# Fytex/Shafa-CD

Hardware: AMD Instinct MI355X
Metric: GiB/s Shannon-Fano encode+decode, 64 MiB blocks, 1/2/4/8 GPUs; bit-exact (higher is better)
Workload: dtype u8

## Files before the change

shafa-cd_amd/csrc/sf_decode.hip:

```cpp
#include <type_traits>
#include "common.hpp"
#include "internal.hpp"

#include <atomic>
#include <mutex>
#include <thread>

#include <algorithm>

#include <stdlib.h>

#include "sfd_common.hpp"
#include "sfd_dp.hpp"
#include "sfd_generic.hpp"

namespace {

typedef __attribute__((address_space(3))) u32 lds_u32;
typedef __attribute__((address_space(3))) u16 lds_u16;
typedef __attribute__((address_space(3))) u8 lds_u8;
template <int LONG> constexpr u32 spec_emask() { return LONG == 2 ? 31u : 15u; }

constexpr int SC_PHW = 16;
constexpr int SC_M = 4;
// ... 725 lines not shown
    if (lds_addr(smem) != 0) __builtin_trap();
    const u32 units = (blk.n_tiles + SC_WTILES - 1) / SC_WTILES;
    u32 first_end = units - 1;
    if (units >= 2 && blk.in_n - (u64)(units - 2) * SC_WTILES * DTILE < (u64)64 * SC_SB + 4) first_end = units - 2;
    if (blockIdx.x > 0) {
        const u32 t_end = first_end * SC_WTILES, t_begin = 1u + (blockIdx.x - 1u) * SF_LINKS;
        if (t_begin < t_end)
            sf_links<LONG>(smem, blk, t_begin, t_end, chunk_entry, chunk_cnt, tile_cnt, tile_guess, tile_exit, tab_bytes, long_bytes);
        return;
    }
    fill_lds16((void *)(smem + SL_LDS_DATA), (const void *)blk.cnt3, 2u << blk.KW);
    if (LONG) {
        u16 *lt = (u16 *)(smem + SL_LDS_DATA + tab_bytes + SL_MISC);
        const u16 *src = LONG == 1 ? blk.longtab : blk.long32;
        if (src) fill_lds16((void *)lt, src, long_bytes);
        else if (threadIdx.x == 0) *lt = 0;
    }
    __syncthreads();
    u32 e0 = first_end ? (u32)tile_exit[(size_t)blk.tile_base + first_end * SC_WTILES - 1] : 0u;
    for (u32 u = first_end; u < units; ++u)
        e0 = sl_region<LONG>(smem, blk, u * SC_WTILES, e0, chunk_entry, chunk_cnt, tile_cnt, tile_guess, tile_exit, tab_bytes);
}

constexpr int ws_row(bool esc) { return CH_BYTES / 4 + (esc ? 3 : 2); }
constexpr int ws_rows_bytes(bool esc)
{
    return 16 + (DEC_THREADS * ws_row(esc) + (esc ? 0 : DEC_THREADS / 16)) * 4;
}
constexpr int WS_MISC = 32;
typedef unsigned int u32x3_t __attribute__((ext_vector_type(3)));
constexpr u32 WS_NST = 4, WS_DROP = 0x7FFFFFF0u;
constexpr int WS_RSRC_FLAGS = 0x00020000, WS_AUX_NT = 2;

template <int LONG, bool ESC>
__global__ __launch_bounds__(DEC_THREADS) void sfd_wstage(const DecBlk *__restrict__ blks, const u8 *__restrict__ chunk_entry,
                                                          const u16 *__restrict__ chunk_cnt, const u64 *__restrict__ tile_off,
                                                          u32 tpw, u32 tab_bytes, u32 cap, u32 long_bytes)
{
    extern __shared__ __attribute__((aligned(16))) u8 smem[];
    const DecBlk blk = blks[blockIdx.y];
    const u32 first_tile = blockIdx.x * tpw;
    if (first_tile >= blk.n_tiles) return;
    if (tile_off[(size_t)blk.tile_base + first_tile] >= blk.n_sym) return;
    const u32 LONGB = LONG ? long_bytes : 0u;
    u32 *rows = (u32 *)(smem + 16);
    constexpr u32 WS_ROW = (u32)ws_row(ESC), tab_off = (u32)ws_rows_bytes(ESC);
    const u16 *lt = (const u16 *)(smem + tab_off + tab_bytes);
    const u32 img_off = tab_off + tab_bytes + LONGB;
    u32 *wsum = (u32 *)(smem + img_off + cap);
    u32 *next = wsum + 4;
    const u32 tid = threadIdx.x, lane = tid & 63, wv = tid >> 6;
    const u32 K1 = blk.K1, K3 = sym3_window(K1);
    const u32 sh = 32 - K1;
    fill_lds16(smem + tab_off, (const void *)blk.sym3, 4u << K3);
    if (LONG) {
        const u16 *src = LONG == 1 ? blk.longtab : blk.long32;
        if (src) fill_lds16((void *)lt, src, LONGB);
        else if (tid == 0) *(u16 *)lt = 0;
    }
    for (u32 i = tid; i < cap / 16; i += DEC_THREADS) *(uint4 *)(smem + img_off + 16 * i) = make_uint4(0, 0, 0, 0);
    bool bad = false;
    if (lds_addr(smem) != 0) __builtin_trap();
    const u32 q2row = 8u * (16u + 4u * (WS_ROW * tid + (ESC ? 0u : tid >> 4))) - 2u;
    const u32 mask4 = ((1u << K3) - 1u) << 2;
    auto fetch16 = [&](const u64 off) -> uint4 {
        if (off + 16 <= blk.in_n) return gload_nt<uint4>(blk.in + off);
        u32 w[4] = {0, 0, 0, 0};
        if (off < blk.in_n) {
            const int nv = (int)(blk.in_n - off);
#pragma unroll
            for (int q = 0; q < 16; ++q)
                if (q < nv) w[q >> 2] |= (u32)gload<u8>(blk.in + off + q) << (8 * (q & 3));
        }
        return make_uint4(w[0], w[1], w[2], w[3]);
    };
    uint4 pf0, pf1;
    u32 pf2[ESC ? 3 : 2] = {};
    auto fetch_ahead = [&](const u64 off) {
        constexpr int NB = ESC ? 12 : 8;
        if (off + NB <= blk.in_n) {
            if constexpr (ESC) {
                const u32x3_t v = __builtin_nontemporal_load((const GLOBAL_AS u32x3_t *)(unsigned long long)(blk.in + off));
                pf2[0] = v.x; pf2[1] = v.y; pf2[2] = v.z;
            } else {
                const uint2 v = gload_nt<uint2>(blk.in + off);
                pf2[0] = v.x; pf2[1] = v.y;
            }
            return;
        }
        u32 w[3] = {0, 0, 0};
        if (off < blk.in_n) {
            const int nv = (int)(blk.in_n - off);
#pragma unroll
            for (int q = 0; q < NB; ++q)
                if (q < nv) w[q >> 2] |= (u32)gload<u8>(blk.in + off + q) << (8 * (q & 3));
        }
#pragma unroll
// ... 55 lines not shown
        u32 pre = incl - cnt, total = 0;
        for (u32 w = 0; w < 4; ++w) { if (w < wv) pre += wsum[w]; total += wsum[w]; }
        const u64 room = blk.n_sym - toff;
        const u32 tot_c = (u32)__builtin_amdgcn_readfirstlane((int)(room < (u64)total ? (u32)room : total));
        u32 want = pre >= tot_c ? 0u : (tot_c - pre < cnt ? tot_c - pre : cnt);
        u32 q2 = q2row + entry;
        const bool by_pos = want == cnt && tile + 1 < blk.n_tiles && nent != spec_emask<LONG>();
        const u32 q2end = q2row + 256u + nent;
        u32 done = 0;
        do {
            u8 *gout = blk.out + toff + done;
            const u32 mis = (u32)((uintptr_t)gout & 15u);
            if (carry_g && (carry_n != mis || carry_g != gout - mis)) {
                if (tid == 0) {
                    uint4 *ip = (uint4 *)(smem + img_off);
                    store_bytes(carry_g, *ip, carry_lo, carry_n);
                    ip[0] = make_uint4(0, 0, 0, 0);
                    ip[1] = make_uint4(0, 0, 0, 0);
                }
                carry_n = 0;
                carry_g = nullptr;
                lds_barrier();
            }
            const u32 capw = cap - 32;
            u32 nxt = tot_c;
            if (mis + (tot_c - done) > capw) {
                if (tid == 0) *next = tot_c;
                lds_barrier();
                if (want && pre >= done && mis + (pre - done) + want > capw) atomicMin(next, pre);
                lds_barrier();
                nxt = (u32)__builtin_amdgcn_readfirstlane((int)*next);
                lds_barrier();
            }
            if (want && pre >= done && pre + want <= nxt) {
                const u32 x = mis + (pre - done);
                u32 wp = img_off + (x & ~3u), nbx = x << 30, acc = 0;
                auto emit = [&](const u32 e) {
                    const u32 sh = nbx >> 27, syms = e & 0xFFFFFFu;
                    acc |= syms << sh;
                    if (__builtin_add_overflow(nbx, e & 0xC0000000u, &nbx)) {
                        __hip_atomic_fetch_or((lds_u32 *)(size_t)wp, acc, __ATOMIC_RELAXED, __HIP_MEMORY_SCOPE_WORKGROUP);
                        wp += 4u;
                        acc = syms >> (32u - sh);
                    }
                };
                auto window4 = [&]() -> u32 {
                    const lds_u32 *pa = (const lds_u32 *)(size_t)((q2 >> 3) & ~3u);
                    return __builtin_amdgcn_alignbit(pa[1], pa[0], q2);
                };
                auto step = [&](const bool tail) {
                    u32 e = *(const lds_u32 *)(size_t)(tab_off + (window4() & mask4));
                    if (ESC && __builtin_expect((e >> 30) == 0, 0)) {
                        const u32 q = q2 + 2u;
                        const lds_u32 *pb = (const lds_u32 *)(size_t)((q >> 3) & ~3u);
                        const u32 win = __builtin_bitreverse32(__builtin_amdgcn_alignbit(pb[1], pb[0], q));
                        u32 e1 = LONG == 1 ? long_code(lt, win) : LONG == 2 ? long_code32(lt, win)
                                           : (u32)gload<u16>(blk.lut13 + (win >> sh));
                        if (e1 == 0) { bad = true; e1 = 1u << 8; }
                        e = (e1 & 0xFFu) | ((e1 >> 8) << 24) | (1u << 30);
                    }
                    u32 n = e >> 30, syms = e & 0xFFFFFFu;
                    if (tail) {
                        n = n < want ? n : want;
                        syms &= (1u << (8 * n)) - 1u;
                    }
                    emit(syms | n << 30);
                    q2 += (e >> 24) & 63u;
// ... 176 lines not shown
    u64 rs = key | 1ull;
    int fails = 0;
    for (int trial = 0; trial < SPEC_TRIALS && fails <= SPEC_MAX_FAILS; ++trial) {
        u64 w[SPEC_WORDS];
        for (u64 &x : w) x = spec_rand(rs);
        if (!spec_trial(w, h.lenlut.data(), h.K1)) ++fails;
    }
    const bool yes = fails <= SPEC_MAX_FAILS;
    std::lock_guard<std::mutex> lk(cmu);
    ckey[slot] = key;
    cval[slot] = yes ? 2 : 1;
    return yes;
}

struct SfdArrays {
    u8 *cfn, *tfn;
    u8 *tent, *cent;
    u16 *ccnt;
    u32 *tcnt;
    u64 *toff;
    u8 *tguess, *texit;
};

enum SfdForm { SFD_MID32, SFD_LONG_ALL, SFD_PACKED12, SFD_PACKED13, SFD_PACKED };

static u32 sfd_tpw(u32 most, u32 max_tiles, int nblocks)
{
    u32 tpw = most;
    while (tpw > 1 && (u64)ceil_div_u64(max_tiles, tpw) * nblocks < 2048) tpw >>= 1;
    return tpw;
}

static void sfd_launch_packed(hipStream_t st, const DecBlk *dblk, int nblocks, u32 max_tiles, SfdForm form, bool esc, bool spec,
                              u32 tabb, u32 long_used, bool all_spec, u32 ws_tab, u32 ws_cap, const SfdArrays &a)
{
    static decltype(&sfd_scan<0>) const scans[3] = {sfd_scan<2>, sfd_scan<1>, sfd_scan<0>};
    static decltype(&sfd_ends<0>) const ends[3] = {sfd_ends<2>, sfd_ends<1>, sfd_ends<0>};
    static decltype(&sfd_sync16<true, false>) const syncs[4] = {sfd_sync16<false, true>, sfd_sync16<true, false, 12>,
                                                                sfd_sync16<true, false, 13>, sfd_sync16<true, false>};
    const int f = form < SFD_PACKED12 ? form : 2;
    const dim3 grid_b((u32)nblocks), wg(DEC_THREADS);
    hipLaunchKernelGGL(sfd_tables, dim3((u32)nblocks, 8), wg, 0, st, dblk);
    if (spec) {
        const size_t lds_scan = (size_t)SC_LDS_ROWS + tabb + SC_MISC + long_used;
        const size_t lds_ends = (size_t)SL_LDS_DATA + tabb + SL_MISC + long_used;
        hipLaunchKernelGGL(scans[f], dim3((u32)ceil_div_u64(max_tiles, SC_TILES), (u32)nblocks), wg, lds_scan, st, dblk, a.cent, a.ccnt,
                           a.tcnt, a.tguess, a.texit, tabb, long_used);
        hipLaunchKernelGGL(ends[f], dim3(1u + (u32)ceil_div_u64(max_tiles, SF_LINKS), (u32)nblocks), wg, lds_ends, st, dblk, a.cent,
                           a.ccnt, a.tcnt, a.tguess, a.texit, tabb, long_used);
    }
    const u32 tpw = all_spec ? 256u : sfd_tpw(4, max_tiles, nblocks);
    const dim3 grid_f((u32)ceil_div_u64(max_tiles, tpw), (u32)nblocks);
    if (form == SFD_MID32) {
        hipLaunchKernelGGL(sfd_sync32, grid_f, wg, 0, st, dblk, a.cfn, a.tfn, tpw);
        hipLaunchKernelGGL(sfd_tiles, grid_b, wg, (size_t)32 * DEC_THREADS + DEC_THREADS, st, dblk, 32u, (const u8 *)a.tfn, a.tent);
        hipLaunchKernelGGL(sfd_countfsm32, grid_f, wg, 0, st, dblk, (const u8 *)a.cfn, (const u8 *)a.tent, a.cent, a.ccnt, a.tcnt, tpw);
    } else {
        constexpr int CSUBS = 4;
        hipLaunchKernelGGL(syncs[form - SFD_LONG_ALL], grid_f, wg, 0, st, dblk, (u64 *)a.cfn, (u64 *)a.tfn, tpw);
        hipLaunchKernelGGL(sfd_tiles16, grid_b, wg, 0, st, dblk, (const u64 *)a.tfn, a.tent);
        hipLaunchKernelGGL((sfd_countfsm<CSUBS>), dim3((u32)ceil_div_u64(max_tiles, tpw * CSUBS), (u32)nblocks), dim3(DEC_THREADS * CSUBS),
                           0, st, dblk, (const u64 *)a.cfn, (const u8 *)a.tent, a.cent, a.ccnt, a.tcnt, tpw);
    }
    hipLaunchKernelGGL(sfd_offsets, grid_b, wg, 0, st, dblk, (const u32 *)a.tcnt, a.toff);
    static decltype(&sfd_wstage<0, false>) const wstages[4] = {sfd_wstage<2, true>, sfd_wstage<1, true>, sfd_wstage<0, true>,
                                                               sfd_wstage<0, false>};
    const u32 tpw_ws = sfd_tpw(16, max_tiles, nblocks);
    const size_t lds_ws = (size_t)ws_rows_bytes(esc) + ws_tab + ws_cap + WS_MISC + long_used;
    hipLaunchKernelGGL(wstages[f == 2 && !esc ? 3 : f], dim3((u32)ceil_div_u64(max_tiles, tpw_ws), (u32)nblocks), wg, lds_ws, st,
                       dblk, (const u8 *)a.cent, (const u16 *)a.ccnt, (const u64 *)a.toff, tpw_ws, ws_tab, ws_cap, long_used);
}

static int sfd_launch_bytemap(hipStream_t st, const DecBlk *dblk, u32 nb, u32 max_tiles, u32 R, u32 l2cap, const SfdArrays &a)
{
    const size_t lds_lut = (size_t)(1u << LUT_MAXK) * 2 + (size_t)l2cap * 2;
    const size_t lds_sync = (size_t)LDS_DATA + (size_t)R * DEC_THREADS + lds_lut + 4 * R + 64;
    const size_t lds_count = lds_sync + DEC_THREADS;
    const size_t lds_write = (size_t)LDS_DATA + lds_lut + 64;
    const size_t lds_tiles = (size_t)R * DEC_THREADS + DEC_THREADS;
    if (lds_tiles > 65536 || lds_sync > 65536) {
        HIP_TRY(hipFuncSetAttribute((const void *)sfd_sync, hipFuncAttributeMaxDynamicSharedMemorySize, (int)lds_sync));
        HIP_TRY(hipFuncSetAttribute((const void *)sfd_count, hipFuncAttributeMaxDynamicSharedMemorySize, (int)lds_count));
        HIP_TRY(hipFuncSetAttribute((const void *)sfd_tiles, hipFuncAttributeMaxDynamicSharedMemorySize, (int)lds_tiles));
    }
    const dim3 grid_t(max_tiles, nb), grid_b(nb), wg(DEC_THREADS);
    hipLaunchKernelGGL(sfd_sync, grid_t, wg, lds_sync, st, dblk, R, l2cap, a.cfn, a.tfn);
    hipLaunchKernelGGL(sfd_tiles, grid_b, wg, lds_tiles, st, dblk, R, (const u8 *)a.tfn, a.tent);
    hipLaunchKernelGGL(sfd_count, grid_t, wg, lds_count, st, dblk, R, l2cap, (const u8 *)a.cfn, (const u8 *)a.tent, a.cent, a.ccnt,
                       a.tcnt);
    hipLaunchKernelGGL(sfd_offsets, grid_b, wg, 0, st, dblk, (const u32 *)a.tcnt, a.toff);
    hipLaunchKernelGGL(sfd_write, grid_t, wg, lds_write, st, dblk, l2cap, (const u8 *)a.cent, (const u16 *)a.ccnt, (const u64 *)a.toff);
    return SHAFA_SUCCESS;
}

int sfdec_launch(Batch *bt, hipStream_t st, int nblocks, const u8 *d_in, const u64 *h_in_off,
                 const u64 *h_in_n, const shafa_code_table *h_tables, const u64 *h_n_symbols, u8 *d_out,
                 const u64 *h_out_off)
{
    if (nblocks <= 0) return SHAFA_SUCCESS;
    if (nblocks > bt->max_blocks) return SHAFA_LACK_OF_MEMORY;

    std::vector<HostTab> tabs(nblocks);
// ... 12 lines not shown
            try { build_host_tab(h_tables[b], tabs[b]); } catch (...) { nomem.store(true); }
        });
        if (nomem.load()) return SHAFA_LACK_OF_MEMORY;
    }
    for (int b = 0; b < nblocks; ++b) {
        HostTab &h = tabs[b];
        bool run = h_n_symbols[b] > 0;
        if (run && (!h.ok || h.empty)) {
            bt->h_hosterr[b] = SHAFA_FILE_UNRECOGNIZABLE;
            run = false;
        }
        if (run && h_in_n[b] == 0) { bt->h_hosterr[b] = SHAFA_FILE_UNRECOGNIZABLE; run = false; }
        if (!run) continue;
        ntiles[b] = (u32)ceil_div_u64(h_in_n[b], DTILE);
        total_tiles += ntiles[b];
        if (ntiles[b] > max_tiles) max_tiles = ntiles[b];
        if (h.lmax > lmax_all) lmax_all = h.lmax;
        tab_bytes += ((h.lut.size() * 2 + 15) & ~(size_t)15) + ((h.trie.size() * 4 + 15) & ~(size_t)15) +
                     ((h.lenlut.size() + 15) & ~(size_t)15) + ((h.lut2.size() * 2 + 16 + 15) & ~(size_t)15) +
                     ((h.lut13.size() * 2 + 15) & ~(size_t)15) + (h.longtab.empty() ? 0 : (size_t)LONG_BYTES) +
                     (h.long32.empty() ? 0 : (size_t)((LONG32_BYTES + 15) & ~15)) + ((h.lenlut32.size() + 15) & ~(size_t)15);
        if (h.lut2.size() > max_l2) max_l2 = (u32)h.lut2.size();
        pair_all = pair_all && h.complete;
        c16_all = c16_all && h.complete16;
        c32_all = c32_all && (h.complete16 || h.complete32);
    }
    if (!total_tiles) return SHAFA_SUCCESS;
    u32 R = 16;
    while (R < lmax_all) R <<= 1;
    if (g_sfd_path >= 1) pair_all = c16_all = c32_all = false;
    const bool long_all = R == 16 && !pair_all && c16_all && lmax_all > (u32)LEN_MAXK;
    const bool packed = R == 16 && ((pair_all && lmax_all <= (u32)LEN_MAXK) || long_all);
    const bool mid32 = !packed && R == 32 && c32_all;
    if (!packed && !mid32 && R < 32) R = 32;

    size_t off = 0;
    const size_t o_blk = off; off += ((size_t)nblocks * sizeof(DecBlk) + 15) & ~(size_t)15;
    const size_t o_rundp = off; off += ((size_t)nblocks * 4 + 15) & ~(size_t)15;
    const size_t o_tab = off; off += tab_bytes;
    const size_t stage_bytes = off;
    const size_t o_tilefn = off; off += (size_t)total_tiles * (R < 8 ? 8 : R); off = (off + 15) & ~(size_t)15;
    const size_t o_tent = off; off += (size_t)total_tiles; off = (off + 15) & ~(size_t)15;
    const size_t o_tcnt = off; off += (size_t)total_tiles * 4; off = (off + 15) & ~(size_t)15;
    const size_t o_toff = off; off += (size_t)total_tiles * 8;
    const size_t o_cent = off; off += (size_t)total_tiles * DEC_THREADS; off = (off + 15) & ~(size_t)15;
    const size_t o_ccnt = off; off += (size_t)total_tiles * DEC_THREADS * 2; off = (off + 15) & ~(size_t)15;
    const bool need_tabs = packed || mid32;
    const size_t o_pair = off; off += (packed && pair_all) ? (size_t)nblocks * (2u << LEN_MAXK) : 0;
    const size_t o_cnt3 = off; off += need_tabs ? (size_t)nblocks * (2u << LEN_MAXK) : 0;
    const size_t o_sym3 = off; off += need_tabs ? (size_t)nblocks * (4u << LEN_MAXK) : 0;
    const size_t o_fsm4 = off; off += need_tabs ? (size_t)nblocks * 16384 : 0;
    const size_t o_fsm1 = off; off += need_tabs ? (size_t)nblocks * 2048 : 0;
    const size_t o_cfn = off; off += packed ? (size_t)total_tiles * DEC_THREADS * 8 : (size_t)total_tiles * R * DEC_THREADS;
    const bool spec_path = (packed || mid32) && g_sfd_speculate != 0;
    std::vector<u32> hblk_kw(nblocks, 0);
    for (int b = 0; b < nblocks; ++b) {
        if (!ntiles[b]) continue;
        u32 n13 = 0;
        if (tabs[b].K1 == 13)
            for (int sy = 0; sy < 256; ++sy) n13 += h_tables[b].len[sy] == 13;
        hblk_kw[b] = scan_window(tabs[b].K1, long_all || mid32, n13);
    }
    u32 long_used = 0;
    if (long_all) {
        u32 gmax = 0;
        for (int b = 0; b < nblocks; ++b)
// ... 18 lines not shown
    u8 *dpar = batch_params_begin(bt, stage_bytes);
    if (!dpar) return SHAFA_LACK_OF_MEMORY;
    ParamsScope pscope(bt, st);
    u8 *hs = (u8 *)batch_stage(bt, bt->par_inline ? st : bt->copy_st, stage_bytes);
    if (!hs) return SHAFA_LACK_OF_MEMORY;
    DecBlk *hb = (DecBlk *)hs;
    size_t tpos = o_tab;
    u32 tbase = 0;
    std::vector<size_t> tab_pos(nblocks, 0);
    for (int b = 0; b < nblocks; ++b) {
        DecBlk &e = hb[b];
        memset(&e, 0, sizeof(e));
        e.in = d_in + h_in_off[b];
        e.out = d_out + h_out_off[b];
        e.in_n = h_in_n[b];
        e.n_sym = h_n_symbols[b];
        e.err = bt->d_err + b;
        e.n_tiles = ntiles[b];
        e.tile_base = tbase;
        e.run_dp = any_spec ? (u32 *)(dpar + o_rundp) + b : nullptr;
        ((u32 *)(hs + o_rundp))[b] = spec_blk[b] ? 0u : 1u;
        e.pairlut = (packed && pair_all) ? ws + o_pair + (size_t)b * (2u << LEN_MAXK) : nullptr;
        e.cnt3 = need_tabs ? (u16 *)(ws + o_cnt3 + (size_t)b * (2u << LEN_MAXK)) : nullptr;
        e.sym3 = need_tabs ? (u32 *)(ws + o_sym3 + (size_t)b * (4u << LEN_MAXK)) : nullptr;
        e.fsm4 = need_tabs ? (u32 *)(ws + o_fsm4 + (size_t)b * 16384) : nullptr;
        e.fsm1 = need_tabs ? (u32 *)(ws + o_fsm1 + (size_t)b * 2048) : nullptr;
        tbase += ntiles[b];
        if (!ntiles[b]) continue;
        HostTab &h = tabs[b];
        e.K = h.K;
        e.K1 = h.K1;
        e.KW = hblk_kw[b];
        e.lmax = h.lmax;
        e.n_states = (u32)(h.trie.size() / 2);
        tab_pos[b] = tpos;
        e.lut2 = (const u16 *)(dpar + tpos);
        e.n_l2 = (u32)h.lut2.size();
        tpos += (h.lut2.size() * 2 + 16 + 15) & ~(size_t)15;
        e.lut13 = (const u16 *)(dpar + tpos);
        tpos += (h.lut13.size() * 2 + 15) & ~(size_t)15;
        if (!h.longtab.empty()) {
            e.longtab = (const u16 *)(dpar + tpos);
            tpos += LONG_BYTES;
        }
        if (!h.long32.empty()) {
            e.long32 = (const u16 *)(dpar + tpos);
            tpos += (LONG32_BYTES + 15) & ~15;
        }
        if (!h.lenlut32.empty()) {
            e.lenlut32 = dpar + tpos;
            tpos += (h.lenlut32.size() + 15) & ~(size_t)15;
        }
        e.lenlut = dpar + tpos;
        if (!e.lenlut32) e.lenlut32 = e.lenlut;
        tpos += (h.lenlut.size() + 15) & ~(size_t)15;
        e.lut = (const u16 *)(dpar + tpos);
        tpos += (h.lut.size() * 2 + 15) & ~(size_t)15;
        e.trie = (const u32 *)(dpar + tpos);
        tpos += (h.trie.size() * 4 + 15) & ~(size_t)15;
    }
    for_blocks_parallel(nblocks, [&](int b) {
        if (!ntiles[b]) return;
        const HostTab &h = tabs[b];
        size_t q = tab_pos[b];
        if (h.lut2.size()) memcpy(hs + q, h.lut2.data(), h.lut2.size() * 2);
        q += (h.lut2.size() * 2 + 16 + 15) & ~(size_t)15;
        memcpy(hs + q, h.lut13.data(), h.lut13.size() * 2);
        q += (h.lut13.size() * 2 + 15) & ~(size_t)15;
        if (!h.longtab.empty()) { memcpy(hs + q, h.longtab.data(), LONG_BYTES); q += LONG_BYTES; }
        if (!h.long32.empty()) { memcpy(hs + q, h.long32.data(), LONG32_BYTES); q += (LONG32_BYTES + 15) & ~15; }
        if (!h.lenlut32.empty()) { memcpy(hs + q, h.lenlut32.data(), h.lenlut32.size()); q += (h.lenlut32.size() + 15) & ~(size_t)15; }
        memcpy(hs + q, h.lenlut.data(), h.lenlut.size());
        q += (h.lenlut.size() + 15) & ~(size_t)15;
        memcpy(hs + q, h.lut.data(), h.lut.size() * 2);
        q += (h.lut.size() * 2 + 15) & ~(size_t)15;
        memcpy(hs + q, h.trie.data(), h.trie.size() * 4);
    });
    if ((rc = batch_params_commit(bt, st, hs, stage_bytes))) return rc;

    const DecBlk *dblk = (const DecBlk *)(dpar + o_blk);
    const SfdArrays arr = {ws + o_cfn, ws + o_tilefn, ws + o_tent, ws + o_cent, (u16 *)(ws + o_ccnt), (u32 *)(ws + o_tcnt),
                           (u64 *)(ws + o_toff), ws + o_tguess, ws + o_texit};
    if (!packed && !mid32) {
        if ((rc = sfd_launch_bytemap(st, dblk, (u32)nblocks, max_tiles, R, (max_l2 + 8) & ~7u, arr))) return rc;
        HIP_TRY(hipGetLastError());
        return pscope.done();
    }
    u32 k1_max = 1, k1_all = 0;
    bool all_spec = any_spec;
    for (int b = 0; b < nblocks; ++b) {
        if (!ntiles[b]) continue;
        if (spec_blk[b] && hblk_kw[b] > k1_max) k1_max = hblk_kw[b];
        k1_all = (k1_all == 0 || k1_all == tabs[b].K1) ? tabs[b].K1 : 0xFFFFFFFFu;
        if (!spec_blk[b]) all_spec = false;
    }
    const SfdForm form = mid32 ? SFD_MID32 : long_all ? SFD_LONG_ALL : k1_all == 12 ? SFD_PACKED12 : k1_all == 13 ? SFD_PACKED13
                                                                                                          : SFD_PACKED;
    u32 ws_tab = 16;
    for (int b = 0; b < nblocks; ++b) {
        const u32 k3 = sym3_window(tabs[b].K1);
        if ((4u << k3) > ws_tab) ws_tab = 4u << k3;
    }
    const bool ws_esc = mid32 || long_all || lmax_all > (u32)SYM3_MAXK;
    u32 ws_cap = 4096, ws_tight = 4096;
    for (int b = 0; b < nblocks; ++b) {
        if (!ntiles[b]) continue;
        const u64 per_tile = ceil_div_u64(h_n_symbols[b], ntiles[b]);
        const u64 c = per_tile + per_tile / 8 + 1024, t = per_tile + per_tile / 32 + 256;
        if (c > ws_cap) ws_cap = (u32)(c > 40960 ? 40960 : c);
        if (t > ws_tight) ws_tight = (u32)(t > 40960 ? 40960 : t);
    }
    {
        const u32 base = (u32)ws_rows_bytes(ws_esc) + ws_tab + long_used + (u32)WS_MISC;
        const u32 most = 65536u - base;
        if (ws_cap > most) ws_cap = most;
        constexpr u32 steps[3] = {20480u, 26880u, 40960u};
        for (u32 k = 0; k < 3; ++k) {
            if (base + ((ws_tight + 15u) & ~15u) <= steps[k]) {
                ws_cap = steps[k] - base;
                if (ws_cap > most) ws_cap = most;
                break;
            }
        }
    }
    ws_cap &= ~15u;
    sfd_launch_packed(st, dblk, nblocks, max_tiles, form, ws_esc, any_spec, 2u << k1_max, long_used, all_spec, ws_tab, ws_cap, arr);
    HIP_TRY(hipGetLastError());
    return pscope.done();
}

#include "sfd_dev.hpp"
```

shafa-cd_amd/csrc/sfd_common.hpp:

```cpp
#pragma once

namespace {


constexpr int DEC_THREADS = 256;
constexpr int CH_BYTES = 32;
constexpr int CH_BITS = CH_BYTES * 8;
constexpr int DTILE = DEC_THREADS * CH_BYTES;
constexpr int HALO_WORDS = 16;
constexpr int DATA_WORDS = DTILE / 4 + HALO_WORDS;
constexpr int LUT_MAXK = 11;
constexpr int LUT2_MAX = 4096;
constexpr int SPEC_MINW = 1;
constexpr int SYM3_MINW = 1;
constexpr int SYM3_MAXK = 12;
constexpr int LDS_DATA = (DATA_WORDS + DATA_WORDS / 8 + 8) * 4;
constexpr int LONG_PFX = 128;
constexpr int LONG_BYTES = 16 + LONG_PFX * 2 + LONG_PFX * 16 * 2;
constexpr int LONG32_BYTES = 16 + LONG_PFX * 2 + LONG_PFX * 2 + 256 * 4 + LONG_PFX * 2;
constexpr int LEN_MAXK = 13;

struct DecBlk {
    const u8 *in;
    u8 *out;
    u64 in_n;
    u64 n_sym;
    int *err;
    const u16 *lut;
    const u16 *lut2;
    const u8 *lenlut;
    u16 *cnt3;
    u32 *sym3;
    u8 *pairlut;
    const u16 *lut13;
    const u32 *trie;
    u32 K;
    u32 K1;
    u32 lmax;
    u32 tile_base;
    u32 n_tiles;
    u32 n_l2;
    u32 n_states;
    u32 KW;
    u32 *fsm4;
    u32 *fsm1;
    const u8 *lenlut32;
    const u16 *long32;
    const u16 *longtab;
    u32 *run_dp;
};

__host__ __device__ __forceinline__ u32 spec_window(u32 K1) { return K1 < (u32)SPEC_MINW ? (u32)SPEC_MINW : K1; }
__host__ __device__ __forceinline__ u32 sym3_window(u32 K1)
{
    const u32 k = K1 < (u32)SYM3_MINW ? (u32)SYM3_MINW : K1;
    return k < (u32)SYM3_MAXK ? k : (u32)SYM3_MAXK;
}
__host__ __device__ __forceinline__ u32 scan_window(u32 K1, bool long_table, u32 n13)
{
    return long_table && K1 == 13 && n13 <= 8 ? 12u : spec_window(K1);
}

constexpr int SPEC_TRIALS = 32, SPEC_MAX_FAILS = 6, SPEC_WORDS = 7;
template <typename LenT, int NB>
__host__ __device__ __forceinline__ u64 spec_key(const LenT *len, const u8 (*bits)[NB])
{
    u64 key = 1469598103934665603ull;
    for (int s = 0; s < 256; ++s) {
        key = (key ^ len[s]) * 1099511628211ull;
        for (u32 q = 0; q < (len[s] + 7) / 8; ++q) key = (key ^ bits[s][q]) * 1099511628211ull;
    }
    return key;
}
__host__ __device__ __forceinline__ u64 spec_rand(u64 &rs)
{
    rs ^= rs << 13; rs ^= rs >> 7; rs ^= rs << 17;
    return rs;
}
__host__ __device__ __forceinline__ bool spec_trial(const u64 *w, const u8 *lenlut, u32 K1)
{
    auto window = [&](u32 pos) -> u32 {
        const u32 wi = pos >> 6, r = pos & 63;
        u64 v = w[wi] << r;
        if (r && wi + 1 < 6) v |= w[wi + 1] >> (64 - r);
        return (u32)(v >> (64 - K1));
    };
    auto len_at = [&](u32 pos) -> u32 { const u32 l = lenlut[window(pos)]; return l ? l : K1 + 1; };
    u64 starts[5] = {0, 0, 0, 0, 0};
    for (u32 pos = 0; pos < 300;) { starts[pos >> 6] |= 1ull << (pos & 63); pos += len_at(pos); }
// ... 84 lines not shown
```

shafa-cd_amd/csrc/sfd_dev.hpp:

```cpp
#pragma once

namespace {

constexpr int SDV_TRIE_PAIRS = 8192;
constexpr int SDV_BIG_PAIRS = 16384;
constexpr int SDV_R_BIG = 64;
constexpr size_t SDV_O_LUT = 0;
constexpr size_t SDV_O_LUT2 = SDV_O_LUT + (2u << LUT_MAXK);
constexpr size_t SDV_O_LEN = SDV_O_LUT2 + LUT2_MAX * 2 + 16;
constexpr size_t SDV_O_L13 = SDV_O_LEN + (1u << LEN_MAXK) + 16;
constexpr size_t SDV_O_LONG = SDV_O_L13 + (2u << LEN_MAXK) + 16;
constexpr size_t SDV_O_TRIE = (SDV_O_LONG + LONG_BYTES + 15) & ~(size_t)15;
constexpr size_t SDV_SLOT = SDV_O_TRIE + (size_t)SDV_TRIE_PAIRS * 8;
constexpr size_t SDV_TABS = (2u << LEN_MAXK) + (4u << LEN_MAXK) + 16384 + 2048 + (2u << LEN_MAXK);

struct SdvHost {
    const u8 *in;
    u8 *out;
    u64 in_cap;
    u64 out_cap;
    u32 tile_base;
    u32 pad;
};

// ... 237 lines not shown
            }
            __syncthreads();
            if (tid < SPEC_TRIALS && !spec_trial(rnd + SPEC_WORDS * tid, lenlut, K1)) atomicAdd(&s_fails, 1u);
            __syncthreads();
            spec = s_fails <= (u32)SPEC_MAX_FAILS;
        }
    }
    __syncthreads();

    u16 *g_lut = (u16 *)(slot + SDV_O_LUT), *g_lut2 = (u16 *)(slot + SDV_O_LUT2), *g_l13 = (u16 *)(slot + SDV_O_L13);
    u8 *g_len = slot + SDV_O_LEN;
    u16 *g_long = (u16 *)(slot + SDV_O_LONG);
    for (u32 i = tid; i < (1u << K); i += 256) g_lut[i] = lut[i];
    for (u32 i = tid; i < s_nl2; i += 256) g_lut2[i] = lut2[i];
    for (u32 i = tid; i < (1u << K1) + 4; i += 256) g_len[i] = lenlut[i];
    for (u32 i = tid; i < (1u << K1) + 2; i += 256)
        g_l13[i] = i < (1u << K1) && lenlut[i] ? (u16)(symlut[i] | ((u32)lenlut[i] << 8)) : (u16)0;
    const bool has_long = packed && lmax > (u32)SYM3_MAXK;
    if (has_long)
        for (u32 i = tid; i < LONG_BYTES / 2; i += 256) g_long[i] = longtab[i];
    if (tid) return;
    e.lut = g_lut;
    e.lut2 = g_lut2;
    e.n_l2 = s_nl2;
    e.lenlut = g_len;
    e.lenlut32 = g_len;
    e.lut13 = g_l13;
    e.trie = trie;
    e.K = K;
    e.K1 = K1;
    e.lmax = lmax;
    e.n_states = nodes;
    e.n_tiles = (u32)((in_n + DTILE - 1) / DTILE);
    if (packed) {
        u8 *tb = po.tabs + (size_t)b * SDV_TABS;
        e.cnt3 = (u16 *)tb;
        e.sym3 = (u32 *)(tb + (2u << LEN_MAXK));
        e.fsm4 = (u32 *)(tb + (6u << LEN_MAXK));
        e.fsm1 = (u32 *)(tb + (6u << LEN_MAXK) + 16384);
        e.longtab = has_long ? g_long : nullptr;
        e.run_dp = po.run_dp ? po.run_dp + b : nullptr;
        if (po.run_dp) po.run_dp[b] = spec ? 0u : 1u;
        if (lmax <= (u32)SYM3_MAXK) {
            e.pairlut = tb + (6u << LEN_MAXK) + 16384 + 2048;
            e.KW = spec_window(K1);
            po.p12[b] = e;
        } else {
            e.KW = scan_window(K1, true, s_n13);
            po.packed[b] = e;
        }
    } else if (big) {
        e.tile_base = 0;
        *po.big = e;
    } else po.bytemap[b] = e;
}

}

int sfdec_launch_dev(Batch *bt, hipStream_t st, int nblocks, const u8 *d_in, const u64 *h_in_off, const u64 *h_in_cap,
                     const u64 *d_in_n, const shafa_code_table *d_tables, const u64 *d_n_symbols, u8 *d_out,
                     const u64 *h_out_off, const u64 *h_out_cap)
{
    if (nblocks <= 0) return SHAFA_SUCCESS;
    if (nblocks > bt->max_blocks) return SHAFA_LACK_OF_MEMORY;
    u64 total = 0;
    u32 max_tiles = 0;
// ... 81 lines not shown
```

shafa-cd_amd/csrc/sfd_dp.hpp:

```cpp
#pragma once


namespace {


__device__ __noinline__ u32 slow_len(const u32 *data, const u32 *trie, u32 p)
{
    u32 node = 0, q = p, depth = 0;
    for (;;) {
        const u32 bit = (data[widx(q >> 5)] >> (31 - (q & 31))) & 1u;
        const u32 nx = trie[2 * node + bit];
        ++q; ++depth;
        if (nx == 0xFFFFFFFFu) return 1;
        if (nx & 0x80000000u) return depth;
        node = nx;
        if (depth >= 255) return 1;
    }
}

__device__ __forceinline__ u32 nib(u64 m, u32 v) { return (u32)(m >> (4 * v)) & 15u; }

__device__ __forceinline__ u64 ring_push(u64 ring, u32 sh4)
{
    const u32 x = (u32)(ring >> (sh4 & 60u));
// ... 44 lines not shown
    }
    return (lo < n && pfx[lo] == key) ? ent[lo * 16 + ((win32 >> 16) & 15u)] : 0u;
}

__device__ __forceinline__ u32 long_code32(const u16 *lt, u32 win32)
{
    const u32 n = lt[0], key = win32 >> 20;
    const u16 *pfx = lt + 8, *root = lt + 8 + LONG_PFX, *nodes = lt + 8 + 2 * LONG_PFX;
    u32 lo = 0, hi = n;
    while (lo < hi) {
        const u32 mid = (lo + hi) >> 1;
        if (pfx[mid] < key) lo = mid + 1; else hi = mid;
    }
    if (lo >= n || pfx[lo] != key) return 0u;
    u32 node = root[lo];
    for (u32 depth = (u32)SYM3_MAXK; depth < 32; ++depth) {
        const u32 c = nodes[2 * node + ((win32 >> (31 - depth)) & 1u)];
        if (c & 0x8000u) return (c & 0xFFu) | ((depth + 1) << 8);
        node = c;
    }
    return 0u;
}

__device__ __forceinline__ void fill_lds16(void *dst, const void *src, u32 bytes)
{
    for (u32 i = threadIdx.x; i < (bytes + 15) / 16; i += blockDim.x)
        ((uint4 *)dst)[i] = gload<uint4>((const uint4 *)src + i);
}

__global__ __launch_bounds__(DEC_THREADS) void sfd_tables(const DecBlk *__restrict__ blks)
{
    const DecBlk blk = blks[blockIdx.x];
    if (!blk.n_tiles) return;
    const u32 T0 = threadIdx.x + blockIdx.y * DEC_THREADS, TS = DEC_THREADS * gridDim.y;
    const u32 K1 = blk.K1, mask = (1u << K1) - 1;
    for (u32 i = T0; blk.pairlut && i < (2u << K1); i += TS)
        blk.pairlut[i] = (u8)((blk.lenlut[i >> 1] - 1u) | ((blk.lenlut[i & mask] - 1u) << 4));
    const u32 K3 = sym3_window(K1);
    const u32 KW = blk.KW, maskw = (1u << KW) - 1;
    for (u32 i = T0; i <= maskw; i += TS) {
        u32 pos = 0, n = 0, l0 = 0;
        for (; n < 7; ++n) {
            const u32 wv = (i << pos) & maskw;
            const u32 L = blk.lut13[KW >= K1 ? wv >> (KW - K1) : wv << (K1 - KW)] >> 8;
            if (L == 0 || L > KW - pos) break;
            if (n == 0) l0 = L;
            pos += L;
        }
        const u32 j = __builtin_bitreverse32(i) >> (32 - KW);
        ((u8 *)blk.cnt3)[j] = (u8)(pos | (n << 5));
        ((u8 *)blk.cnt3)[(1u << KW) + j] = (u8)l0;
    }
    for (u32 i = T0; i < (1u << K3); i += TS) {
        u32 pos = 0, n = 0, syms = 0;
        for (; n < 3; ++n) {
            const u32 e = blk.lut13[K3 >= K1 ? (((i << pos) & ((1u << K3) - 1u)) >> (K3 - K1)) : (((i << (K1 - K3)) << pos) & mask)];
            const u32 L = e >> 8;
            if (L == 0 || L > K3 - pos) break;
            syms |= (e & 0xFFu) << (8 * n);
            pos += L;
        }
        blk.sym3[__builtin_bitreverse32(i) >> (32 - K3)] = syms | (pos << 24) | (n << 30);
    }
    for (u32 i = T0; i < blk.n_states * 16; i += TS) {
        u32 node = i >> 4, done = 0;
        for (int b = 3; b >= 0; --b) {
            const u32 c = blk.trie[2 * node + ((i >> b) & 1u)];
            if (c & 0x80000000u) { ++done; node = 0; } else node = c;
        }
        blk.fsm4[i] = (node * 64u) | (done << 16);
    }
    for (u32 i = T0; i < blk.n_states * 2; i += TS) {
        const u32 c = blk.trie[i];
        blk.fsm1[i] = (c & 0x80000000u) ? (1u << 16) : (c * 64u);
    }
}

template <bool PAIR, bool LONG, int K1T = 0>
__global__ __launch_bounds__(DEC_THREADS) void sfd_sync16(const DecBlk *__restrict__ blks,
                                                          u64 *__restrict__ chunkfn, u64 *__restrict__ tilefn, u32 tpw)
{
    __shared__ __attribute__((aligned(16))) u8 smem[LDS_DATA + (PAIR ? 2 : 1) * (1 << LEN_MAXK) + 64 + (LONG ? LONG_BYTES : 0)];
    if (dp_skipped_early(blks + blockIdx.y)) return;
    const DecBlk blk = blks[blockIdx.y];
    if (blockIdx.x * tpw >= blk.n_tiles) return;
    u32 *data = (u32 *)smem;
// ... 440 lines not shown
```

shafa-cd_amd/csrc/sfd_host_tables.hpp:

```cpp
#pragma once

namespace {
struct HostTab {
    std::vector<u32> trie;
    std::vector<u16> lut, lut2, lut13;
    std::vector<u8> lenlut;
    std::vector<u16> longtab;
    std::vector<u16> long32;
    std::vector<u8> lenlut32;
    u32 K, K1, lmax;
    bool ok, empty, complete, complete16, complete32;
};

void build_host_tab(const shafa_code_table &t, HostTab &h)
{
    h.trie.assign(2, 0xFFFFFFFFu);
    h.ok = true;
    h.complete = false;
    h.complete16 = false;
    h.complete32 = false;
    h.lmax = 0;
    for (int s = 0; s < 256; ++s) h.lmax = t.len[s] > h.lmax ? t.len[s] : h.lmax;
    h.empty = h.lmax == 0;
    h.K = h.lmax < (u32)LUT_MAXK ? (h.lmax ? h.lmax : 1) : (u32)LUT_MAXK;
    h.lut.assign((size_t)1 << h.K, 0);
    h.K1 = h.lmax < (u32)LEN_MAXK ? (h.lmax ? h.lmax : 1) : (u32)LEN_MAXK;
    h.lenlut.assign(((size_t)1 << h.K1) + 4, 0);
    h.lut13.assign(((size_t)1 << h.K1) + 2, 0);
    auto code_of = [&](int s) {
        u64 code = 0;
        const u32 L = t.len[s] < 32 ? t.len[s] : 32;
        for (u32 q = 0; q < L; ++q) code = (code << 1) | ((t.bits[s][q >> 3] >> (7 - (q & 7))) & 1u);
        return (u32)code;
    };
    for (int s = 0; s < 256 && h.ok; ++s) {
        const u32 L = t.len[s];
        if (!L) continue;
        u32 node = 0;
        for (u32 q = 0; q < L; ++q) {
            const u32 bit = (t.bits[s][q >> 3] >> (7 - (q & 7))) & 1u;
            u32 &slot = h.trie[2 * node + bit];
            if (q == L - 1) {
                if (slot != 0xFFFFFFFFu) { h.ok = false; break; }
                slot = 0x80000000u | (u32)s;
            } else {
                if (slot == 0xFFFFFFFFu) {
                    slot = (u32)(h.trie.size() / 2);
                    h.trie.push_back(0xFFFFFFFFu);
                    h.trie.push_back(0xFFFFFFFFu);
                } else if (slot & 0x80000000u) { h.ok = false; break; }
                node = h.trie[2 * node + bit];
            }
        }
        if (h.ok && L <= h.K) {
            const u32 code = code_of(s);
            const u32 lo = code << (h.K - L), cnt = 1u << (h.K - L);
            for (u32 i = 0; i < cnt; ++i) h.lut[lo + i] = (u16)(s | (L << 8));
        }
        if (h.ok && L <= h.K1) {
            const u32 code = code_of(s);
            const u32 lo = code << (h.K1 - L), cnt = 1u << (h.K1 - L);
            memset(h.lenlut.data() + lo, (int)L, cnt);
            if (!h.lut13.empty())
                for (u32 i = 0; i < cnt; ++i) h.lut13[lo + i] = (u16)(s | (L << 8));
        }
    }
    if (!h.ok) return;
    h.complete = h.lmax <= (u32)LEN_MAXK;
    for (size_t i = 0; h.complete && i < ((size_t)1 << h.K1); ++i) h.complete = h.lenlut[i] != 0;
    if (h.lmax <= 16) {
        u64 kraft = 0;
        for (int s = 0; s < 256; ++s) if (t.len[s]) kraft += 1ull << (16 - t.len[s]);
        h.complete16 = kraft == 65536;
    }
    if (h.lmax > (u32)SYM3_MAXK && h.lmax <= 32) {
        u64 kraft = 0;
        for (int s = 0; s < 256; ++s) if (t.len[s]) kraft += 1ull << (32 - t.len[s]);
        h.complete32 = kraft == (1ull << 32);
    }
    if (h.complete32) {
        h.long32.assign(LONG32_BYTES / 2, 0);
        struct Item { u32 key, node; };
        std::vector<Item> roots;
        std::vector<Item> frontier{{0u, 0u}};
        for (int depth = 0; depth < SYM3_MAXK; ++depth) {
            std::vector<Item> next;
            for (const Item &it : frontier)
                for (u32 b = 0; b < 2; ++b) {
                    const u32 c = h.trie[2 * it.node + b];
                    if (c != 0xFFFFFFFFu && !(c & 0x80000000u)) next.push_back({(it.key << 1) | b, c});
                }
            frontier.swap(next);
        }
        roots = frontier;
        std::sort(roots.begin(), roots.end(), [](const Item &a, const Item &b) { return a.key < b.key; });
        std::vector<u32> order;
        std::vector<int> newid(h.trie.size() / 2, -1);
        if (roots.size() > (size_t)LONG_PFX) h.complete32 = false;
        for (size_t g = 0; g < roots.size() && h.complete32; ++g) {
            std::vector<u32> q{roots[g].node};
            for (size_t qi = 0; qi < q.size(); ++qi) {
                const u32 nd = q[qi];
// ... 90 lines not shown
```

Before: 882.8.

## Add single-symbol LUT walk variant to the write stage for short-code tables

Adds a write-stage kernel variant that decodes one symbol per LDS lookup using a compact 2-byte bit-reversed table, instead of the 4-byte multi-symbol (up to three symbols) table. A host heuristic picks it when the code is complete, has no escapes, and few table windows would pack multiple symbols. The new walk builds output bytes with perm/alignbyte, writes whole interior words with plain stores, and uses atomics only at the edges. This shrinks the LDS table and cuts atomic traffic, but does one lookup per symbol and takes on more complex tail handling.

```diff
diff --git a/shafa-cd_amd/csrc/sf_decode.hip b/shafa-cd_amd/csrc/sf_decode.hip
--- a/shafa-cd_amd/csrc/sf_decode.hip
+++ b/shafa-cd_amd/csrc/sf_decode.hip
@@ -781,7 +781,92 @@
 constexpr u32 WS_NST = 4, WS_DROP = 0x7FFFFFF0u;
 constexpr int WS_RSRC_FLAGS = 0x00020000, WS_AUX_NT = 2;
 
-template <int LONG, bool ESC>
+__device__ __forceinline__ void ws_walk1(const u32 tab_off, const u32 mask2, const u32 xa, u32 q2, const u32 q2end, u32 want,
+                                         const bool by_pos)
+{
+    auto window2 = [&]() -> u32 {
+        const lds_u32 *pa = (const lds_u32 *)(size_t)((q2 >> 3) & ~3u);
+        return __builtin_amdgcn_alignbit(pa[1], pa[0], q2);
+    };
+    auto look = [&](const u32 w) -> u32 { return *(const lds_u16 *)(size_t)(tab_off + (w & mask2)); };
+    auto image_or = [](const u32 at, const u32 v) {
+        __hip_atomic_fetch_or((lds_u32 *)(size_t)at, v, __ATOMIC_RELAXED, __HIP_MEMORY_SCOPE_WORKGROUP);
+    };
+    if (by_pos) {
+        constexpr u32 N = 3, F = 4, WPG = F * N / 4;
+        const u32 s = (0u - xa) & 3u;
+        u32 ptr = ((xa + 3u) & ~3u) - 4u;
+        u32 L = 0, Lp = 0, Ep = 0;
+        auto group = [&](auto first_group) -> bool {
+            constexpr bool FIRST = decltype(first_group)::value;
+            u32 x0 = 0, x1 = 0, ub = 0;
+#pragma unroll
+            for (u32 f = 0; f < F; ++f) {
+                if (!((int)q2 < (int)q2end)) {
+                    if (f == 0) {
+                        if (!FIRST) {
+                            image_or(ptr + 4u * (WPG - 1u), Ep);
+                            image_or(ptr + 4u * WPG, __builtin_amdgcn_alignbyte(0u, Lp, s));
+                        }
+                    } else {
+                        const u32 at = ptr + 4u * (f * N >> 2);
+                        image_or(at, __builtin_amdgcn_alignbyte(L, Lp, s));
+                        image_or(at + 4u, __builtin_amdgcn_alignbyte(0u, L, s));
+                    }
+                    return false;
+                }
+                if (f == 0 && !FIRST) {
+                    *(lds_u32 *)(size_t)(ptr + 4u * (WPG - 1u)) = Ep;
+                    ptr += 4u * WPG;
+                }
+                u32 w;
+                if ((f & 1u) == 0) {
+                    const lds_u32 *pa = (const lds_u32 *)(size_t)((q2 >> 3) & ~3u);
+                    const u32 w0 = pa[0], w1 = pa[1], w2 = pa[2];
+                    w = x0 = __builtin_amdgcn_alignbit(w1, w0, q2);
+                    x1 = __builtin_amdgcn_alignbit(w2, w1, q2);
+                } else
+                    w = __builtin_amdgcn_alignbit(x1, x0, ub);
+                u32 ua = 0;
+#pragma unroll
+                for (u32 i = 0; i < N; ++i) {
+                    const u32 k = f * N + i, b = k & 3u;
+                    const u32 e = look(w >> ua);
+                    ua += e >> 8;
+                    L = __builtin_amdgcn_perm(e, L, b == 0 ? 0x0C0C0C04u : b == 1 ? 0x0C0C0400u : b == 2 ? 0x0C040100u : 0x04020100u);
+                    if (b == 3u) {
+                        const u32 E = __builtin_amdgcn_alignbyte(L, Lp, s), at = ptr + 4u * (k >> 2);
+                        Lp = L;
+                        if (FIRST && k == 3u) image_or(at, E);
+                        else if (k == F * N - 1u) Ep = E;
+                        else *(lds_u32 *)(size_t)at = E;
+                    }
+                }
+                q2 += ua;
+                ub = ua;
+            }
+            return true;
+        };
+        if (group(std::true_type{}))
+            while (group(std::false_type{})) {}
+        return;
+    }
+    u32 wp = xa & ~3u, nb = 8u * (xa & 3u), acc = 0;
+    for (; want; --want) {
+        const u32 e = look(window2());
+        q2 += e >> 8;
+        acc |= (e & 0xFFu) << nb;
+        nb += 8u;
+        if (nb == 32u) {
+            image_or(wp, acc);
+            wp += 4u;
+            acc = nb = 0;
+        }
+    }
+    if (nb) image_or(wp, acc);
+}
+
+template <int LONG, bool ESC, bool ONE = false>
 __global__ __launch_bounds__(DEC_THREADS) void sfd_wstage(const DecBlk *__restrict__ blks, const u8 *__restrict__ chunk_entry,
                                                           const u16 *__restrict__ chunk_cnt, const u64 *__restrict__ tile_off,
                                                           u32 tpw, u32 tab_bytes, u32 cap, u32 long_bytes)
@@ -801,7 +886,9 @@
     const u32 tid = threadIdx.x, lane = tid & 63, wv = tid >> 6;
     const u32 K1 = blk.K1, K3 = sym3_window(K1);
     const u32 sh = 32 - K1;
-    fill_lds16(smem + tab_off, (const void *)blk.sym3, 4u << K3);
+    static_assert(!ONE || (LONG == 0 && !ESC), "the one-code walk has no escapes");
+    constexpr bool one = ONE;
+    fill_lds16(smem + tab_off, (const void *)blk.sym3, (one ? 2u : 4u) << K3);
     if (LONG) {
         const u16 *src = LONG == 1 ? blk.longtab : blk.long32;
         if (src) fill_lds16((void *)lt, src, LONGB);
@@ -810,8 +897,8 @@
     for (u32 i = tid; i < cap / 16; i += DEC_THREADS) *(uint4 *)(smem + img_off + 16 * i) = make_uint4(0, 0, 0, 0);
     bool bad = false;
     if (lds_addr(smem) != 0) __builtin_trap();
-    const u32 q2row = 8u * (16u + 4u * (WS_ROW * tid + (ESC ? 0u : tid >> 4))) - 2u;
-    const u32 mask4 = ((1u << K3) - 1u) << 2;
+    const u32 q2row = 8u * (16u + 4u * (WS_ROW * tid + (ESC ? 0u : tid >> 4))) - (one ? 1u : 2u);
+    const u32 mask4 = ((1u << K3) - 1u) << (one ? 1 : 2);
     auto fetch16 = [&](const u64 off) -> uint4 {
         if (off + 16 <= blk.in_n) return gload_nt<uint4>(blk.in + off);
         u32 w[4] = {0, 0, 0, 0};
@@ -933,7 +1020,10 @@
                 nxt = (u32)__builtin_amdgcn_readfirstlane((int)*next);
                 lds_barrier();
             }
-            if (want && pre >= done && pre + want <= nxt) {
+            const bool mine = want && pre >= done && pre + want <= nxt;
+            if constexpr (ONE) {
+                if (mine) ws_walk1(tab_off, mask4, img_off + mis + (pre - done), q2, q2end, want, by_pos);
+            } else if (mine) {
                 const u32 x = mis + (pre - done);
                 u32 wp = img_off + (x & ~3u), nbx = x << 30, acc = 0;
                 auto emit = [&](const u32 e) {
@@ -1176,7 +1266,7 @@
 }
 
 static void sfd_launch_packed(hipStream_t st, const DecBlk *dblk, int nblocks, u32 max_tiles, SfdForm form, bool esc, bool spec,
-                              u32 tabb, u32 long_used, bool all_spec, u32 ws_tab, u32 ws_cap, const SfdArrays &a)
+                              u32 tabb, u32 long_used, bool all_spec, u32 ws_tab, u32 ws_cap, const SfdArrays &a, bool one = false)
 {
     static decltype(&sfd_scan<0>) const scans[3] = {sfd_scan<2>, sfd_scan<1>, sfd_scan<0>};
     static decltype(&sfd_ends<0>) const ends[3] = {sfd_ends<2>, sfd_ends<1>, sfd_ends<0>};
@@ -1207,11 +1297,11 @@
                            0, st, dblk, (const u64 *)a.cfn, (const u8 *)a.tent, a.cent, a.ccnt, a.tcnt, tpw);
     }
     hipLaunchKernelGGL(sfd_offsets, grid_b, wg, 0, st, dblk, (const u32 *)a.tcnt, a.toff);
-    static decltype(&sfd_wstage<0, false>) const wstages[4] = {sfd_wstage<2, true>, sfd_wstage<1, true>, sfd_wstage<0, true>,
-                                                               sfd_wstage<0, false>};
+    static decltype(&sfd_wstage<0, false>) const wstages[5] = {sfd_wstage<2, true>, sfd_wstage<1, true>, sfd_wstage<0, true>,
+                                                               sfd_wstage<0, false>, sfd_wstage<0, false, true>};
     const u32 tpw_ws = sfd_tpw(16, max_tiles, nblocks);
     const size_t lds_ws = (size_t)ws_rows_bytes(esc) + ws_tab + ws_cap + WS_MISC + long_used;
-    hipLaunchKernelGGL(wstages[f == 2 && !esc ? 3 : f], dim3((u32)ceil_div_u64(max_tiles, tpw_ws), (u32)nblocks), wg, lds_ws, st,
+    hipLaunchKernelGGL(wstages[one ? 4 : f == 2 && !esc ? 3 : f], dim3((u32)ceil_div_u64(max_tiles, tpw_ws), (u32)nblocks), wg, lds_ws, st,
                        dblk, (const u8 *)a.cent, (const u16 *)a.ccnt, (const u64 *)a.toff, tpw_ws, ws_tab, ws_cap, long_used);
 }
 
@@ -1290,6 +1380,10 @@
     const bool long_all = R == 16 && !pair_all && c16_all && lmax_all > (u32)LEN_MAXK;
     const bool packed = R == 16 && ((pair_all && lmax_all <= (u32)LEN_MAXK) || long_all);
     const bool mid32 = !packed && R == 32 && c32_all;
+    const bool ws_esc = mid32 || long_all || lmax_all > (u32)SYM3_MAXK;
+    bool ws_one = !ws_esc;
+    for (int b = 0; b < nblocks; ++b)
+        if (ntiles[b] && !tabs[b].one) ws_one = false;
     if (!packed && !mid32 && R < 32) R = 32;
 
     size_t off = 0;
@@ -1374,6 +1468,7 @@
         e.K1 = h.K1;
         e.KW = hblk_kw[b];
         e.lmax = h.lmax;
+        e.one = ws_one;
         e.n_states = (u32)(h.trie.size() / 2);
         tab_pos[b] = tpos;
         e.lut2 = (const u16 *)(dpar + tpos);
@@ -1440,10 +1535,9 @@
                                                                                                           : SFD_PACKED;
     u32 ws_tab = 16;
     for (int b = 0; b < nblocks; ++b) {
-        const u32 k3 = sym3_window(tabs[b].K1);
-        if ((4u << k3) > ws_tab) ws_tab = 4u << k3;
-    }
-    const bool ws_esc = mid32 || long_all || lmax_all > (u32)SYM3_MAXK;
+        const u32 k3 = sym3_window(tabs[b].K1), tb = (ws_one ? 2u : 4u) << k3;
+        if (tb > ws_tab) ws_tab = tb;
+    }
     u32 ws_cap = 4096, ws_tight = 4096;
     for (int b = 0; b < nblocks; ++b) {
         if (!ntiles[b]) continue;
@@ -1466,7 +1560,7 @@
         }
     }
     ws_cap &= ~15u;
-    sfd_launch_packed(st, dblk, nblocks, max_tiles, form, ws_esc, any_spec, 2u << k1_max, long_used, all_spec, ws_tab, ws_cap, arr);
+    sfd_launch_packed(st, dblk, nblocks, max_tiles, form, ws_esc, any_spec, 2u << k1_max, long_used, all_spec, ws_tab, ws_cap, arr, ws_one);
     HIP_TRY(hipGetLastError());
     return pscope.done();
 }
diff --git a/shafa-cd_amd/csrc/sfd_common.hpp b/shafa-cd_amd/csrc/sfd_common.hpp
--- a/shafa-cd_amd/csrc/sfd_common.hpp
+++ b/shafa-cd_amd/csrc/sfd_common.hpp
@@ -47,6 +47,7 @@
     const u8 *lenlut32;
     const u16 *long32;
     const u16 *longtab;
+    u32 one;
     u32 *run_dp;
 };
 
@@ -55,6 +56,20 @@
 {
     const u32 k = K1 < (u32)SYM3_MINW ? (u32)SYM3_MINW : K1;
     return k < (u32)SYM3_MAXK ? k : (u32)SYM3_MAXK;
+}
+__host__ __forceinline__ bool sym1_pays(const u8 *lenlut, u32 K1)
+{
+    if (K1 > 10) return false;
+    const u32 mask = (1u << K1) - 1u;
+    u32 n = 0;
+    for (u32 i = 0; i <= mask; ++i)
+        for (u32 pos = 0, c = 0; c < 3; ++c) {
+            const u32 L = lenlut[(i << pos) & mask];
+            if (L == 0 || L > K1 - pos) break;
+            pos += L;
+            ++n;
+        }
+    return 5u * n <= (7u << K1);
 }
 __host__ __device__ __forceinline__ u32 scan_window(u32 K1, bool long_table, u32 n13)
 {
diff --git a/shafa-cd_amd/csrc/sfd_dev.hpp b/shafa-cd_amd/csrc/sfd_dev.hpp
--- a/shafa-cd_amd/csrc/sfd_dev.hpp
+++ b/shafa-cd_amd/csrc/sfd_dev.hpp
@@ -293,6 +293,7 @@
     e.lmax = lmax;
     e.n_states = nodes;
     e.n_tiles = (u32)((in_n + DTILE - 1) / DTILE);
+    e.one = 0;
     if (packed) {
         u8 *tb = po.tabs + (size_t)b * SDV_TABS;
         e.cnt3 = (u16 *)tb;
diff --git a/shafa-cd_amd/csrc/sfd_dp.hpp b/shafa-cd_amd/csrc/sfd_dp.hpp
--- a/shafa-cd_amd/csrc/sfd_dp.hpp
+++ b/shafa-cd_amd/csrc/sfd_dp.hpp
@@ -100,6 +100,7 @@
 {
     const DecBlk blk = blks[blockIdx.x];
     if (!blk.n_tiles) return;
+    const bool one = blk.one != 0;
     const u32 T0 = threadIdx.x + blockIdx.y * DEC_THREADS, TS = DEC_THREADS * gridDim.y;
     const u32 K1 = blk.K1, mask = (1u << K1) - 1;
     for (u32 i = T0; blk.pairlut && i < (2u << K1); i += TS)
@@ -119,7 +120,11 @@
         ((u8 *)blk.cnt3)[j] = (u8)(pos | (n << 5));
         ((u8 *)blk.cnt3)[(1u << KW) + j] = (u8)l0;
     }
-    for (u32 i = T0; i < (1u << K3); i += TS) {
+    for (u32 i = T0; one && i < (1u << K3); i += TS) {
+        const u32 e = blk.lut13[i];
+        ((u16 *)blk.sym3)[__builtin_bitreverse32(i) >> (32 - K3)] = (u16)(e >> 8 ? e : 1u << 8);
+    }
+    for (u32 i = T0; !one && i < (1u << K3); i += TS) {
         u32 pos = 0, n = 0, syms = 0;
         for (; n < 3; ++n) {
             const u32 e = blk.lut13[K3 >= K1 ? (((i << pos) & ((1u << K3) - 1u)) >> (K3 - K1)) : (((i << (K1 - K3)) << pos) & mask)];
diff --git a/shafa-cd_amd/csrc/sfd_host_tables.hpp b/shafa-cd_amd/csrc/sfd_host_tables.hpp
--- a/shafa-cd_amd/csrc/sfd_host_tables.hpp
+++ b/shafa-cd_amd/csrc/sfd_host_tables.hpp
@@ -10,6 +10,7 @@
     std::vector<u8> lenlut32;
     u32 K, K1, lmax;
     bool ok, empty, complete, complete16, complete32;
+    bool one;
 };
 
 void build_host_tab(const shafa_code_table &t, HostTab &h)
@@ -19,6 +20,7 @@
     h.complete = false;
     h.complete16 = false;
     h.complete32 = false;
+    h.one = false;
     h.lmax = 0;
     for (int s = 0; s < 256; ++s) h.lmax = t.len[s] > h.lmax ? t.len[s] : h.lmax;
     h.empty = h.lmax == 0;
@@ -68,6 +70,7 @@
     if (!h.ok) return;
     h.complete = h.lmax <= (u32)LEN_MAXK;
     for (size_t i = 0; h.complete && i < ((size_t)1 << h.K1); ++i) h.complete = h.lenlut[i] != 0;
+    h.one = h.complete && h.lmax <= (u32)SYM3_MAXK && sym1_pays(h.lenlut.data(), h.K1);
     if (h.lmax <= 16) {
         u64 kraft = 0;
         for (int s = 0; s < 256; ++s) if (t.len[s]) kraft += 1ull << (16 - t.len[s]);
```

Measured after the change: 904.0, median of 6. 1.02x the previous value.
